# dotchen/LAV

Hardware: NVIDIA H100
Metric: agent_frames_per_s (higher is better)
Workload: dtype fp16 storage, fp32 accumulate (wgmma f16 / mma.sync f16; saturating stores)

## Files before the change

include/lav_b200.h:

```cpp
#ifndef LAV_B200_H
#define LAV_B200_H

#include <stddef.h>
#include <stdint.h>

#ifdef __cplusplus
extern "C" {
#endif

#define LAVB_ABI_VERSION 3

int lavb_abi_version(void);
const char* lavb_last_error(void);
int lavb_device_cc(void);

enum { LAVB_F32 = 0, LAVB_BF16 = 1, LAVB_F16 = 2 };
int lavb_h16_dtype(void);

int lavb_paint(const float* d_pts, int n, int pt_stride,
               const float* d_sem, int ncam, int c_in, int h, int w,
               long long s_cam, long long s_c, long long s_y, long long s_x,
               const float* h_cams, int mode,
               float* d_out, int out_stride, int out_col0, int copy_cols, void* stream);

// ... 160 lines not shown
int lavb_pillar_scatter_max(const float* d_h, const int* d_cell, int m, int c, long long n_cells,
                            float* d_canvas, int* d_argmax, void* stream);
int lavb_pillar_scatter_max_bwd(const float* d_gcanvas, const int* d_argmax, const int* d_cell, int m, int c,
                                float* d_gh, void* stream);

typedef struct {
  const void* in; int in_dtype; int n, hin, win, cin, in_cstride, in_coff;
  void* out; int out_dtype; int hout, wout, cout, out_cstride, out_coff;
  int hog, wog;
  int in_sy, in_sx, out_sy, out_sx, out_oy, out_ox;
  int ntaps; int dy[16]; int dx[16];
  const float* w; const float* bias; const float* scale; const float* shift;
  const void* res; int res_dtype; int res_cstride, res_coff;
  int pre_relu, post_relu, sigmoid;
  int d2s_nout;
} lavb_conv_desc;
int lavb_conv_taps(const lavb_conv_desc* h_desc, void* stream);

int lavb_deconv3x3s2_small(const void* d_in, int dtype, int n, int h, int w, int in_cstride, int groups, int cin_g,
                           const float* d_w, const float* d_bias, const int* h_n_out, const int* h_sigmoid,
                           float* const* h_out_ptrs, void* stream);

int lavb_pool2_affine_relu(const void* d_in, int dtype, int n, int hin, int win, int c, int in_cstride, int in_coff,
                           const float* d_scale, const float* d_shift,
                           void* d_out, int out_cstride, int out_coff, void* stream);

int lavb_rgb_normalize(const void* d_rgb, int src_is_u8_nhwc, int n, int h, int w, void* d_out, int out_dtype,
                       void* stream);

int lavb_stem7x7s2_u8(const void* d_img, int batch, int ncam, int h, int cam_w, const void* d_w, const float* d_bias,
                      const float* h_mean, const float* h_std, void* d_out, void* stream);
int lavb_maxpool3x3s2_nhwc(const void* d_in, int n, int h, int w, int c, void* d_out, void* stream);

size_t lavb_det_peaks_workspace_bytes(int batch, int ncls);
int lavb_det_peaks(const float* d_center, const float* d_box, const float* d_ori, int batch, int h, int w, int ncls,
                   float min_score, int max_det, float* d_packed, void* d_workspace, void* stream);

int lavb_crop_bilinear(const void* d_feat, int dtype, int b, int h, int w, int c, const int* d_frame_idx,
                       const float* d_theta, int k, int crop, void* d_out, void* stream);
int lavb_crop_bilinear_u8(const uint8_t* d_map, int b, int c, int h, int w, const int* d_frame_idx, const float* d_theta,
                          int k, int crop, float* d_out, void* stream);
int lavb_crop_bilinear_bwd(const float* d_gout, int b, int h, int w, int c, const int* d_frame_idx, const float* d_theta,
                           int k, int crop, float* d_gfeat, void* stream);

int lavb_convert(const void* d_src, int src_dtype, void* d_dst, int dst_dtype, long long count, void* stream);

int lavb_conv_umma(const lavb_conv_desc* h_desc, void* stream);

int lavb_conv7x7s2_umma(const void* d_in, int n, int h, int w, int cin, const void* d_w, const float* d_bias, void* d_out,
                        void* stream);

int lavb_conv3x3_umma(const void* d_in, int n, int h, int w, int cin, int stride, const void* d_w, int cout, const float* d_bias,
                      const float* d_scale, const float* d_shift, int pre_relu, void* d_out, void* stream);

typedef struct lavb_conv_pair_desc {
  const void* in; void* out; const void* res;
  int n, h, w, c, dil, post_relu;
  const void* w1; const float* bias1;
  const void* w2; const float* shift2;
} lavb_conv_pair_desc;
int lavb_conv_pair_umma(const lavb_conv_pair_desc* h_desc, void* stream);
int lavb_conv_pair_set_trace(void* d_buf, int tiles_per_cta);

int lavb_erf_stem(const void* d_rgb_u8, int n, int h, int w, const float* h_w27x16, const float* h_scale16,
                  const float* h_shift16, void* d_out, int out_dtype, void* stream);

int lavb_erf_down16(const void* d_in, void* d_out, int n, int h, int w, const float* d_w9, const float* d_st, void* stream);

int lavb_erf_nb16(const void* d_in, void* d_out, int n, int h, int w, const float* d_w4, const float* d_st, void* stream);

int lavb_cast_gru(const float* d_embd, int n, const float* d_wih_t, const float* d_whh_t, const float* d_bih, const float* d_bhh,
                  const float* d_wmlp, const float* d_bmlp, int ncmd, int steps, float* d_out, void* stream);

#ifdef __cplusplus
}
#endif
#endif
```

lav_b200/capi.py:

```python
import ctypes as C
import os

_HERE = os.path.dirname(os.path.abspath(__file__))
LIB_PATH = os.path.join(_HERE, "_lib", "liblavb200.so")

F32, BF16, F16 = 0, 1, 2


class LavbError(RuntimeError):
    pass


class ConvDesc(C.Structure):
    _fields_ = [
        ("inp", C.c_void_p), ("in_dtype", C.c_int), ("n", C.c_int), ("hin", C.c_int), ("win", C.c_int), ("cin", C.c_int),
        ("in_cstride", C.c_int), ("in_coff", C.c_int),
        ("out", C.c_void_p), ("out_dtype", C.c_int), ("hout", C.c_int), ("wout", C.c_int), ("cout", C.c_int),
        ("out_cstride", C.c_int), ("out_coff", C.c_int),
        ("hog", C.c_int), ("wog", C.c_int),
        ("in_sy", C.c_int), ("in_sx", C.c_int), ("out_sy", C.c_int), ("out_sx", C.c_int), ("out_oy", C.c_int), ("out_ox", C.c_int),
        ("ntaps", C.c_int), ("dy", C.c_int * 16), ("dx", C.c_int * 16),
        ("w", C.c_void_p), ("bias", C.c_void_p), ("scale", C.c_void_p), ("shift", C.c_void_p),
        ("res", C.c_void_p), ("res_dtype", C.c_int), ("res_cstride", C.c_int), ("res_coff", C.c_int),
        ("pre_relu", C.c_int), ("post_relu", C.c_int), ("sigmoid", C.c_int), ("d2s_nout", C.c_int),
# ... 84 lines not shown
    "lavb_agent_nav_state_bytes": (C.c_size_t, []),
    "lavb_agent_nav_front": (C.c_int, [C.c_int, C.c_void_p, C.c_void_p, C.c_int, C.c_void_p, C.c_void_p, C.c_void_p, C.c_void_p,
                                       C.c_void_p, C.c_void_p, C.c_void_p, C.c_void_p, C.c_void_p]),
    "lavb_agent_nav_update": (C.c_int, [C.c_int, C.c_void_p, C.c_void_p, C.c_void_p, C.c_void_p, C.c_void_p, C.c_void_p]),
    "lavb_stack_job_poses": (C.c_int, [C.c_void_p, C.c_int, C.c_int, C.c_int, C.c_int, C.c_longlong, C.c_void_p, C.c_void_p,
                                       C.c_void_p]),
    "lavb_agent_view_scratch_bytes": (C.c_size_t, [C.c_int]),
    "lavb_agent_view": (C.c_int, [C.c_void_p, C.c_void_p, C.c_void_p, C.c_int, C.c_longlong, C.c_int, C.c_void_p, C.c_int, C.c_int,
                                  C.c_void_p, C.c_void_p, C.c_void_p, C.c_void_p, C.c_int, C.c_void_p, C.c_void_p, C.c_int, C.c_int,
                                  C.c_void_p, C.c_void_p, C.c_int, C.c_void_p, C.c_void_p, C.POINTER(ViewConfig), C.c_void_p,
                                  C.c_size_t, C.c_void_p, C.c_void_p]),
    "lavb_roof_filter": (C.c_int, [C.c_void_p, C.c_int, C.c_int, C.c_int, C.c_longlong, C.c_void_p, C.c_longlong, C.c_void_p, C.c_int,
                                   C.c_void_p]),
    "lavb_stack_sweep": (C.c_int, [C.c_void_p, C.c_int, C.c_int, C.c_void_p, C.c_float, C.c_float, C.c_int, C.c_int, C.c_int,
                                   C.c_void_p, C.c_void_p]),
    "lavb_pillar_workspace_bytes": (C.c_size_t, [C.c_int, C.c_int, C.c_int]),
    "lavb_pillar_forward": (C.c_int, [C.c_void_p, C.c_int, C.c_int, C.c_void_p, C.c_void_p, C.c_int,
                                      C.c_float, C.c_float, C.c_float, C.c_float, C.c_float, C.c_int, C.c_int,
                                      C.c_void_p, C.c_void_p, C.c_void_p, C.c_int, C.c_void_p, C.c_void_p, C.c_void_p, C.c_int,
                                      C.c_void_p, C.c_int, C.c_void_p, C.c_void_p]),
    "lavb_pillar_sorted_workspace_bytes": (C.c_size_t, [C.c_int, C.c_int, C.c_int, C.c_longlong]),
    "lavb_pillar_forward_sorted": (C.c_int, [C.c_void_p, C.c_int, C.c_int, C.c_void_p, C.c_void_p, C.c_int,
                                             C.c_float, C.c_float, C.c_float, C.c_float, C.c_float, C.c_int, C.c_int,
                                             C.c_void_p, C.c_void_p, C.c_void_p, C.c_int, C.c_void_p, C.c_void_p, C.c_void_p, C.c_int,
                                             C.c_void_p, C.c_int, C.c_void_p, C.c_void_p]),
    "lavb_pillar_decorate": (C.c_int, [C.c_void_p, C.c_int, C.c_int, C.c_void_p, C.c_void_p, C.c_int,
                                       C.c_float, C.c_float, C.c_float, C.c_float, C.c_float, C.c_int, C.c_int,
                                       C.c_void_p, C.c_void_p, C.c_void_p, C.c_void_p, C.c_void_p]),
    "lavb_pillar_scatter_max": (C.c_int, [C.c_void_p, C.c_void_p, C.c_int, C.c_int, C.c_longlong, C.c_void_p, C.c_void_p,
                                          C.c_void_p]),
    "lavb_pillar_scatter_max_bwd": (C.c_int, [C.c_void_p, C.c_void_p, C.c_void_p, C.c_int, C.c_int, C.c_void_p, C.c_void_p]),
    "lavb_conv_taps": (C.c_int, [C.POINTER(ConvDesc), C.c_void_p]),
    "lavb_pool2_affine_relu": (C.c_int, [C.c_void_p, C.c_int, C.c_int, C.c_int, C.c_int, C.c_int, C.c_int, C.c_int,
                                         C.c_void_p, C.c_void_p, C.c_void_p, C.c_int, C.c_int, C.c_void_p]),
    "lavb_rgb_normalize": (C.c_int, [C.c_void_p, C.c_int, C.c_int, C.c_int, C.c_int, C.c_void_p, C.c_int, C.c_void_p]),
    "lavb_convert": (C.c_int, [C.c_void_p, C.c_int, C.c_void_p, C.c_int, C.c_longlong, C.c_void_p]),
    "lavb_stem7x7s2_u8": (C.c_int, [C.c_void_p, C.c_int, C.c_int, C.c_int, C.c_int, C.c_void_p, C.c_void_p, C.c_void_p, C.c_void_p,
                                    C.c_void_p, C.c_void_p]),
    "lavb_erf_stem": (C.c_int, [C.c_void_p, C.c_int, C.c_int, C.c_int, C.c_void_p, C.c_void_p, C.c_void_p, C.c_void_p, C.c_int, C.c_void_p]),
    "lavb_erf_down16": (C.c_int, [C.c_void_p, C.c_void_p, C.c_int, C.c_int, C.c_int, C.c_void_p, C.c_void_p, C.c_void_p]),
    "lavb_erf_nb16": (C.c_int, [C.c_void_p, C.c_void_p, C.c_int, C.c_int, C.c_int, C.c_void_p, C.c_void_p, C.c_void_p]),
    "lavb_conv_pair_umma": (C.c_int, [C.c_void_p, C.c_void_p]),
    "lavb_maxpool3x3s2_nhwc": (C.c_int, [C.c_void_p, C.c_int, C.c_int, C.c_int, C.c_int, C.c_void_p, C.c_void_p]),
    "lavb_det_peaks_workspace_bytes": (C.c_size_t, [C.c_int, C.c_int]),
    "lavb_det_peaks": (C.c_int, [C.c_void_p, C.c_void_p, C.c_void_p, C.c_int, C.c_int, C.c_int, C.c_int, C.c_float, C.c_int,
                                 C.c_void_p, C.c_void_p, C.c_void_p]),
    "lavb_crop_bilinear": (C.c_int, [C.c_void_p, C.c_int, C.c_int, C.c_int, C.c_int, C.c_int, C.c_void_p, C.c_void_p, C.c_int,
                                     C.c_int, C.c_void_p, C.c_void_p]),
    "lavb_crop_bilinear_u8": (C.c_int, [C.c_void_p, C.c_int, C.c_int, C.c_int, C.c_int, C.c_void_p, C.c_void_p, C.c_int, C.c_int,
                                        C.c_void_p, C.c_void_p]),
    "lavb_cast_gru": (C.c_int, [C.c_void_p, C.c_int, C.c_void_p, C.c_void_p, C.c_void_p, C.c_void_p, C.c_void_p, C.c_void_p, C.c_int,
                                C.c_int, C.c_void_p, C.c_void_p]),
    "lavb_conv_pair_set_trace": (C.c_int, [C.c_void_p, C.c_int]),
    "lavb_crop_bilinear_bwd": (C.c_int, [C.c_void_p, C.c_int, C.c_int, C.c_int, C.c_int, C.c_void_p, C.c_void_p, C.c_int, C.c_int,
                                         C.c_void_p, C.c_void_p]),
    "lavb_deconv3x3s2_small": (C.c_int, [C.c_void_p, C.c_int, C.c_int, C.c_int, C.c_int, C.c_int, C.c_int, C.c_int, C.c_void_p,
                                         C.c_void_p, C.c_void_p, C.c_void_p, C.c_void_p, C.c_void_p]),
    "lavb_conv_umma": (C.c_int, [C.POINTER(ConvDesc), C.c_void_p]),
    "lavb_conv7x7s2_umma": (C.c_int, [C.c_void_p, C.c_int, C.c_int, C.c_int, C.c_int, C.c_void_p, C.c_void_p, C.c_void_p,
                                      C.c_void_p]),
    "lavb_conv3x3_umma": (C.c_int, [C.c_void_p, C.c_int, C.c_int, C.c_int, C.c_int, C.c_int, C.c_void_p, C.c_int, C.c_void_p,
                                    C.c_void_p, C.c_void_p, C.c_int, C.c_void_p, C.c_void_p]),
}

_lib = None


def exported_symbols():
    return sorted(_SIGS)


def lib():
    global _lib
    if _lib is None:
        if not os.path.exists(LIB_PATH):
            raise LavbError(f"{LIB_PATH} is missing — run `python -m lav_b200.build` (or __graft_entry__.build()); "
                            "lav_b200 has no CPU fallback")
        handle = C.CDLL(LIB_PATH)
        for name, (res, args) in _SIGS.items():
            fn = getattr(handle, name)
            fn.restype = res
            fn.argtypes = args
        if handle.lavb_abi_version() != 3:
            raise LavbError("liblavb200.so ABI version mismatch")
        _lib = handle
    return _lib


def h16_code():
    return lib().lavb_h16_dtype()


def check(code, what):
    if code != 0:
        raise LavbError(f"{what} failed ({code}): {lib().lavb_last_error().decode()}")
```

lav_b200/csrc/sm90.cuh:

```cuda
#pragma once
#include <cuda.h>
#include <cudaTypedefs.h>
#include "common.cuh"

namespace lavb {
namespace sm90 {

__device__ __forceinline__ uint32_t smem_u32(const void* p) { return (uint32_t)__cvta_generic_to_shared(p); }

__device__ __forceinline__ void proxy_fence_async() { asm volatile("fence.proxy.async.shared::cta;" ::: "memory"); }
__device__ __forceinline__ void bar_sync(int id, int threads) { asm volatile("bar.sync %0, %1;" ::"r"(id), "r"(threads) : "memory"); }

__device__ __forceinline__ void mbar_init(uint32_t bar, uint32_t count) {
  asm volatile("mbarrier.init.shared::cta.b64 [%0], %1;" ::"r"(bar), "r"(count));
}
__device__ __forceinline__ void mbar_expect_tx(uint32_t bar, uint32_t bytes) {
  asm volatile("mbarrier.arrive.expect_tx.shared::cta.b64 _, [%0], %1;" ::"r"(bar), "r"(bytes) : "memory");
}
__device__ __forceinline__ void mbar_arrive(uint32_t bar) {
  asm volatile("mbarrier.arrive.shared::cta.b64 _, [%0];" ::"r"(bar) : "memory");
}
__device__ __forceinline__ void mbar_wait(uint32_t bar, uint32_t parity) {
  uint32_t done;
  do {
    asm volatile(
        "{\n\t.reg .pred p;\n\t"
        "mbarrier.try_wait.parity.shared::cta.b64 p, [%1], %2;\n\t"
        "selp.u32 %0, 1, 0, p;\n\t}"
        : "=r"(done) : "r"(bar), "r"(parity) : "memory");
  } while (!done);
}
__device__ __forceinline__ void tma_load_4d(uint32_t dst, const CUtensorMap* map, uint32_t bar, int c0, int c1, int c2, int c3) {
  asm volatile(
      "cp.async.bulk.tensor.4d.shared::cluster.global.mbarrier::complete_tx::bytes [%0], [%1, {%3, %4, %5, %6}], [%2];"
      ::"r"(dst), "l"(reinterpret_cast<uint64_t>(map)), "r"(bar), "r"(c0), "r"(c1), "r"(c2), "r"(c3) : "memory");
}
__device__ __forceinline__ void tma_load_2d(uint32_t dst, const CUtensorMap* map, uint32_t bar, int c0, int c1) {
  asm volatile(
      "cp.async.bulk.tensor.2d.shared::cluster.global.mbarrier::complete_tx::bytes [%0], [%1, {%3, %4}], [%2];"
      ::"r"(dst), "l"(reinterpret_cast<uint64_t>(map)), "r"(bar), "r"(c0), "r"(c1) : "memory");
}
__device__ __forceinline__ void mbar_arrive(uint32_t bar, uint32_t count) {
  asm volatile("mbarrier.arrive.shared::cta.b64 _, [%0], %1;" ::"r"(bar), "r"(count) : "memory");
}

__device__ __forceinline__ void tma_store_4d(const CUtensorMap* map, uint32_t src, int c0, int c1, int c2, int c3) {
  asm volatile("cp.async.bulk.tensor.4d.global.shared::cta.bulk_group [%0, {%2, %3, %4, %5}], [%1];"
               ::"l"(reinterpret_cast<uint64_t>(map)), "r"(src), "r"(c0), "r"(c1), "r"(c2), "r"(c3) : "memory");
}
__device__ __forceinline__ void bulk_commit() { asm volatile("cp.async.bulk.commit_group;" ::: "memory"); }
template <int N> __device__ __forceinline__ void bulk_wait_read() { asm volatile("cp.async.bulk.wait_group.read %0;" ::"n"(N) : "memory"); }
template <int N> __device__ __forceinline__ void bulk_wait() { asm volatile("cp.async.bulk.wait_group %0;" ::"n"(N) : "memory"); }

inline PFN_cuTensorMapEncodeTiled_v12000 get_encode() {
  static PFN_cuTensorMapEncodeTiled_v12000 fn = nullptr;
  if (!fn) {
    void* p = nullptr;
    cudaDriverEntryPointQueryResult q;
    if (cudaGetDriverEntryPoint("cuTensorMapEncodeTiled", &p, cudaEnableDefault, &q) == cudaSuccess && q == cudaDriverEntryPointSuccess)
      fn = reinterpret_cast<PFN_cuTensorMapEncodeTiled_v12000>(p);
  }
  return fn;
}

__device__ __forceinline__ uint64_t desc_sw128(uint32_t saddr) {
  const uint32_t lo = ((saddr & 0x3FFFFu) >> 4) | (1u << 16);
  const uint32_t hi = (1024u >> 4) | (1u << 30);
  return (uint64_t)lo | ((uint64_t)hi << 32);
}

__device__ __forceinline__ void wgmma_fence() { asm volatile("wgmma.fence.sync.aligned;" ::: "memory"); }
__device__ __forceinline__ void wgmma_commit() { asm volatile("wgmma.commit_group.sync.aligned;" ::: "memory"); }
template <int N> __device__ __forceinline__ void wgmma_wait() { asm volatile("wgmma.wait_group.sync.aligned %0;" ::"n"(N) : "memory"); }
template <int N> __device__ __forceinline__ void acc_fence(float (&d)[N]) {
#pragma unroll
  for (int i = 0; i < N; ++i) asm volatile("" : "+f"(d[i])::"memory");
}

template <int N> __device__ void wgmma(float (&d)[N / 2], uint64_t a, uint64_t b, uint32_t accumulate);

#define LAVB_WG_R0 "%0, %1, %2, %3, %4, %5, %6, %7, %8, %9, %10, %11, %12, %13, %14, %15"
#define LAVB_WG_R1 "%16, %17, %18, %19, %20, %21, %22, %23, %24, %25, %26, %27, %28, %29, %30, %31"
#define LAVB_WG_R2 "%32, %33, %34, %35, %36, %37, %38, %39, %40, %41, %42, %43, %44, %45, %46, %47"
#define LAVB_WG_R3 "%48, %49, %50, %51, %52, %53, %54, %55, %56, %57, %58, %59, %60, %61, %62, %63"
#define LAVB_WG_R4 "%64, %65, %66, %67, %68, %69, %70, %71, %72, %73, %74, %75, %76, %77, %78, %79"
#define LAVB_WG_R5 "%80, %81, %82, %83, %84, %85, %86, %87, %88, %89, %90, %91, %92, %93, %94, %95"
#define LAVB_WG_R6 "%96, %97, %98, %99, %100, %101, %102, %103, %104, %105, %106, %107, %108, %109, %110, %111"
#define LAVB_WG_R7 "%112, %113, %114, %115, %116, %117, %118, %119, %120, %121, %122, %123, %124, %125, %126, %127"
#define LAVB_WG_D4(i) "+f"(d[i]), "+f"(d[i + 1]), "+f"(d[i + 2]), "+f"(d[i + 3])
#define LAVB_WG_D16(i) LAVB_WG_D4(i), LAVB_WG_D4(i + 4), LAVB_WG_D4(i + 8), LAVB_WG_D4(i + 12)
#define LAVB_WGMMA(N, REGS, IA, IB, IP, ...)                                                                         \
  template <> __device__ __forceinline__ void wgmma<N>(float (&d)[N / 2], uint64_t a, uint64_t b, uint32_t accumulate) { \
    asm volatile(                                                                                                      \
        "{\n\t.reg .pred p;\n\t"                                                                                       \
        "setp.ne.b32 p, %" #IP ", 0;\n\t"                                                                              \
        "wgmma.mma_async.sync.aligned.m64n" #N "k16.f32." LAVB_H16_PTX "." LAVB_H16_PTX " "                            \
        "{" REGS "}, %" #IA ", %" #IB ", p, 1, 1, 0, 0;\n\t}"                                                          \
        : __VA_ARGS__                                                                                                  \
        : "l"(a), "l"(b), "r"(accumulate));                                                                            \
  }
LAVB_WGMMA(32, LAVB_WG_R0, 16, 17, 18, LAVB_WG_D16(0))
// ... 29 lines not shown
```

lav_b200/csrc/stem_umma.cu:

```cuda
#include "sm90.cuh"

namespace lavb {
namespace cmajor {

using namespace sm90;

constexpr int kTile = 16;
constexpr int kBlockK = 64;
constexpr int kColBytes = kTile * kBlockK * 2;
constexpr int kThreads = 288;
constexpr int kEpiPitch = 64 * 2 + 16;
constexpr int kEpiPx = 64;
constexpr int kEpiBytes = kEpiPx * kEpiPitch;
constexpr int kMaxCout = 256;
constexpr int kSmemCap = 227 * 1024;

template <int KS, int S, int CO, int SC>
struct Cfg {
  static constexpr int kCols = S == 1 ? kTile + KS - 1 : kTile + (KS - 1) / 2;
  static constexpr int kBoxBytes = kCols * kColBytes;
  static constexpr int kPBytes = SC * S * kBoxBytes;
  static constexpr int kWBytes = CO * kBlockK * 2;
  static constexpr int kN = CO == 64 ? 8 * kTile : 16 * kTile;
  static constexpr int kCtrl = 16 * 32 + 3 * kMaxCout * 4;
  static constexpr int kFixed = 1024  + 2 * kEpiBytes + kCtrl;
  static constexpr int kPStages = kPBytes <= 40 * 1024 ? 3 : 2;
  static constexpr int kWFit = (kSmemCap - kFixed - kPStages * kPBytes) / kWBytes;
  static constexpr int kWStages = kWFit < 12 ? kWFit : 12;
  static constexpr int kSmem = kFixed + kPStages * kPBytes + kWStages * kWBytes;
  static_assert(kWStages >= 3 && kPStages + kWStages <= 32 && kSmem <= kSmemCap, "shared-memory plan");
};

struct Args {
  int ho, wo, cout, kchunks, tiles_x, tiles_per_img, ncol, num_tiles;
  int pre_bias;
  int pre_relu;
  float shift0;
  h16* out;
  const float* bias; const float* scale; const float* shift;
};

template <int KS, int S, int CO, int SC>
__global__ void __launch_bounds__(kThreads, 1) conv_cmajor_kernel(const __grid_constant__ CUtensorMap tmap_x,
                                                                  const __grid_constant__ CUtensorMap tmap_w,
                                                                  const __grid_constant__ Args p) {
  using C = Cfg<KS, S, CO, SC>;
  constexpr int kPStages = C::kPStages, kWStages = C::kWStages, kPBytes = C::kPBytes, kWBytes = C::kWBytes;
  constexpr int kBoxBytes = C::kBoxBytes, kN = C::kN;
  extern __shared__ uint8_t smem_raw[];
  const uint32_t base = (smem_u32(smem_raw) + 1023u) & ~1023u;
  uint8_t* gen = smem_raw + (base - smem_u32(smem_raw));
  const uint32_t wring = base + kPStages * kPBytes;
  const uint32_t epi = wring + kWStages * kWBytes;
  const uint32_t ctrl = epi + 2 * kEpiBytes;
  const uint32_t p_full = ctrl, p_empty = ctrl + 8 * kPStages, w_full = ctrl + 16 * kPStages, w_empty = w_full + 8 * kWStages;
  float* ep_b = reinterpret_cast<float*>(gen + (ctrl - base) + 16 * 32);
  float* ep_s = ep_b + kMaxCout;
  float* ep_t = ep_s + kMaxCout;

  const int warp = threadIdx.x >> 5, lane = threadIdx.x & 31;
  if (threadIdx.x == 0) {
    asm volatile("prefetch.tensormap [%0];" ::"l"(reinterpret_cast<uint64_t>(&tmap_x)) : "memory");
    asm volatile("prefetch.tensormap [%0];" ::"l"(reinterpret_cast<uint64_t>(&tmap_w)) : "memory");
    for (int s = 0; s < kPStages; ++s) { mbar_init(p_full + 8 * s, 1); mbar_init(p_empty + 8 * s, 8); }
    for (int s = 0; s < kWStages; ++s) { mbar_init(w_full + 8 * s, 1); mbar_init(w_empty + 8 * s, 8); }
    asm volatile("fence.mbarrier_init.release.cluster;" ::: "memory");
  }
  for (int c = threadIdx.x; c < p.cout; c += blockDim.x) {
    const float b = p.bias ? __ldg(p.bias + c) : 0.f;
    const float sc = p.scale ? __ldg(p.scale + c) : 1.f;
    const float sh = p.shift ? __ldg(p.shift + c) : p.shift0;
    ep_b[c] = b;
    ep_s[c] = sc;
    ep_t[c] = p.pre_bias ? sh : fmaf(b, sc, sh);
  }
  __syncthreads();
  const int nkg = p.kchunks / SC;

  if (warp == 8) {
    if (lane == 0) {
      int ps = 0, ws = 0; uint32_t pph = 0, wph = 0;
      for (int tile = blockIdx.x; tile < p.num_tiles; tile += gridDim.x) {
        const int col = tile % p.ncol, sp = tile / p.ncol;
        const int img = sp / p.tiles_per_img, r = sp - img * p.tiles_per_img;
        const int y0 = (r / p.tiles_x) * S * kTile - KS / 2, x0 = (r % p.tiles_x) * S * kTile - KS / 2;
        for (int kg = 0; kg < nkg; ++kg) {
          for (int ky = 0; ky < KS; ++ky) {
            mbar_wait(p_empty + 8 * ps, pph ^ 1);
            const uint32_t sp_at = base + ps * kPBytes;
            mbar_expect_tx(p_full + 8 * ps, kPBytes);
            for (int c = 0; c < SC; ++c)
              for (int par = 0; par < S; ++par)
                tma_load_4d(sp_at + (c * S + par) * kBoxBytes, &tmap_x, p_full + 8 * ps, (kg * SC + c) * kBlockK, y0 + ky,
                            x0 + par, img);
            if (++ps == kPStages) { ps = 0; pph ^= 1; }
            for (int kx = 0; kx < KS; ++kx) {
              for (int c = 0; c < SC; ++c) {
                mbar_wait(w_empty + 8 * ws, wph ^ 1);
                mbar_expect_tx(w_full + 8 * ws, kWBytes);
                tma_load_2d(wring + ws * kWBytes, &tmap_w, w_full + 8 * ws, (kg * SC + c) * kBlockK,
                            (KS * ky + kx) * p.cout + col * CO);
                if (++ws == kWStages) { ws = 0; wph ^= 1; }
              }
            }
          }
        }
      }
    }
    return;
  }

  const int wg = warp >> 2;
  const int wtid = threadIdx.x & 127;
  uint8_t* ep = gen + (epi - base) + wg * kEpiBytes;
  const uint32_t a_off = CO == 128 ? wg * (64 * kBlockK * 2) : 0;
  const uint32_t b_off = CO == 64 ? wg * (8 * kColBytes) : 0;
  const int co = 16 * (warp & 3) + (lane >> 2);
  int ps = 0, ws = 0; uint32_t pph = 0, wph = 0;
  float acc[kN / 2];
  for (int tile = blockIdx.x; tile < p.num_tiles; tile += gridDim.x) {
    for (int kg = 0; kg < nkg; ++kg) {
      for (int ky = 0; ky < KS; ++ky) {
        mbar_wait(p_full + 8 * ps, pph);
        const uint32_t sp_at = base + ps * kPBytes + b_off;
        for (int kx = 0; kx < KS; ++kx) {
#pragma unroll
          for (int c = 0; c < SC; ++c) {
            mbar_wait(w_full + 8 * ws, wph);
            const uint64_t a_desc = desc_sw128(wring + ws * kWBytes + a_off);
            const uint64_t b_desc = desc_sw128(sp_at + (c * S + kx % S) * kBoxBytes + (kx / S) * kColBytes);
            const bool first = (kg | ky | kx | c) == 0;
            wgmma_fence();
#pragma unroll
            for (int k = 0; k < kBlockK / 16; ++k)
              wgmma<kN>(acc, a_desc + (uint64_t)(2 * k), b_desc + (uint64_t)(2 * k), (!first || k) ? 1u : 0u);
            wgmma_commit();
            wgmma_wait<1>();
            if (lane == 0 && !first) {
              mbar_arrive(w_empty + 8 * (ws ? ws - 1 : kWStages - 1));
              if (kx == 0 && c == 0) mbar_arrive(p_empty + 8 * (ps ? ps - 1 : kPStages - 1));
            }
            if (++ws == kWStages) { ws = 0; wph ^= 1; }
          }
        }
        if (++ps == kPStages) { ps = 0; pph ^= 1; }
      }
    }
    wgmma_wait<0>();
    acc_fence(acc);
    if (lane == 0) {
      mbar_arrive(w_empty + 8 * (ws ? ws - 1 : kWStages - 1));
      mbar_arrive(p_empty + 8 * (ps ? ps - 1 : kPStages - 1));
    }

    const int col = tile % p.ncol, sp = tile / p.ncol;
    const int img = sp / p.tiles_per_img, r = sp - img * p.tiles_per_img;
    const int oy0 = (r / p.tiles_x) * kTile, ox0 = (r % p.tiles_x) * kTile + (CO == 64 ? 8 * wg : 0);
    const int ch0 = col * CO + (CO == 128 ? 64 * wg : 0);
    const float b0 = ep_b[ch0 + co], b1 = ep_b[ch0 + co + 8];
    const float s0 = ep_s[ch0 + co], s1 = ep_s[ch0 + co + 8];
    const float t0 = ep_t[ch0 + co], t1 = ep_t[ch0 + co + 8];
#pragma unroll
    for (int pass = 0; pass < kN / kEpiPx; ++pass) {
      bar_sync(1 + wg, 128);
#pragma unroll
      for (int i = 8 * pass; i < 8 * pass + 8; ++i)
#pragma unroll
        for (int e = 0; e < 2; ++e) {
          const int px = 8 * i + 2 * (lane & 3) + e - kEpiPx * pass;
          uint8_t* row = ep + px * kEpiPitch;
          float x0 = acc[4 * i + e], x1 = acc[4 * i + 2 + e];
          if (p.pre_bias) { x0 += b0; x1 += b1; }
          if (p.pre_relu) { x0 = fmaxf(x0, 0.f); x1 = fmaxf(x1, 0.f); }
          x0 = fmaf(x0, s0, t0);
          x1 = fmaf(x1, s1, t1);
          *reinterpret_cast<h16*>(row + 2 * co) = float2h16(x0);
          *reinterpret_cast<h16*>(row + 2 * (co + 8)) = float2h16(x1);
        }
      bar_sync(1 + wg, 128);
#pragma unroll
      for (int j = 0; j < kEpiPx * 64 * 2 / 16 / 128; ++j) {
        const int q = wtid + 128 * j, px = q >> 3, piece = q & 7;
        const int n = kEpiPx * pass + px, oy = oy0 + n % kTile, ox = ox0 + n / kTile;
        if (oy < p.ho && ox < p.wo)
          *reinterpret_cast<uint4*>(p.out + (((long long)img * p.ho + oy) * p.wo + ox) * p.cout + ch0 + 8 * piece) =
              *reinterpret_cast<const uint4*>(ep + px * kEpiPitch + 16 * piece);
      }
    }
  }
}

static int encode_maps(const char* who, const void* d_in, int n, int h, int w, int cin, int ks, int s, const void* d_w, int cout,
                       int co, CUtensorMap* tmap_x, CUtensorMap* tmap_w) {
  auto encode = get_encode();
  LAVB_CHECK_ARG(encode != nullptr, "%s: cuTensorMapEncodeTiled not available from the driver", who);
  {
    const int cols = s == 1 ? kTile + ks - 1 : kTile + (ks - 1) / 2;
    cuuint64_t dims[4] = {(cuuint64_t)cin, (cuuint64_t)h, (cuuint64_t)w, (cuuint64_t)n};
    cuuint64_t strides[3] = {(cuuint64_t)w * cin * 2, (cuuint64_t)cin * 2, (cuuint64_t)h * w * cin * 2};
    cuuint32_t box[4] = {(cuuint32_t)kBlockK, (cuuint32_t)(s * kTile), (cuuint32_t)(s * cols), 1};
    cuuint32_t estr[4] = {1, (cuuint32_t)s, (cuuint32_t)s, 1};
    CUresult r = encode(tmap_x, LAVB_TMAP_H16, 4, const_cast<void*>(d_in), dims, strides, box, estr,
                        CU_TENSOR_MAP_INTERLEAVE_NONE, CU_TENSOR_MAP_SWIZZLE_128B, CU_TENSOR_MAP_L2_PROMOTION_L2_256B,
                        CU_TENSOR_MAP_FLOAT_OOB_FILL_NONE);
    LAVB_CHECK_ARG(r == CUDA_SUCCESS, "%s: cuTensorMapEncodeTiled(x) failed with %d", who, (int)r);
  }
  {
    cuuint64_t dims[2] = {(cuuint64_t)cin, (cuuint64_t)ks * ks * cout};
    cuuint64_t strides[1] = {(cuuint64_t)cin * 2};
    cuuint32_t box[2] = {(cuuint32_t)kBlockK, (cuuint32_t)co};
    cuuint32_t estr[2] = {1, 1};
    CUresult r = encode(tmap_w, LAVB_TMAP_H16, 2, const_cast<void*>(d_w), dims, strides, box, estr,
                        CU_TENSOR_MAP_INTERLEAVE_NONE, CU_TENSOR_MAP_SWIZZLE_128B, CU_TENSOR_MAP_L2_PROMOTION_L2_256B,
                        CU_TENSOR_MAP_FLOAT_OOB_FILL_NONE);
    LAVB_CHECK_ARG(r == CUDA_SUCCESS, "%s: cuTensorMapEncodeTiled(w) failed with %d", who, (int)r);
  }
  return 0;
}

template <int KS, int S, int CO, int SC>
static int launch(const CUtensorMap& tmap_x, const CUtensorMap& tmap_w, const Args& a, void* stream) {
  constexpr int smem = Cfg<KS, S, CO, SC>::kSmem;
  LAVB_CUDA_OK(ensure_dyn_smem((const void*)conv_cmajor_kernel<KS, S, CO, SC>, smem));
  conv_cmajor_kernel<KS, S, CO, SC><<<min(a.num_tiles, kNumSMs), kThreads, smem, (cudaStream_t)stream>>>(tmap_x, tmap_w, a);
  LAVB_LAUNCH_OK();
  return 0;
}

static int check_operands(const char* who, const void* d_in, int n, int h, int w, int cin, int taps, const void* d_w, int cout,
                          const float* bias, const float* scale, const float* shift, const void* d_out, int ho, int wo, int co) {
  const auto al = [](const void* q, int a) { return reinterpret_cast<uintptr_t>(q) % a == 0; };
  LAVB_CHECK_ARG(al(d_in, 16) && al(d_w, 16) && al(d_out, 16), "%s: d_in, d_w and d_out must be 16 B aligned", who);
  LAVB_CHECK_ARG(al(bias, 4) && al(scale, 4) && al(shift, 4), "%s: bias, scale and shift must be 4 B aligned", who);
  LAVB_CHECK_ARG((long long)n * ceil_div(ho, kTile) * ceil_div(wo, kTile) * (cout / co) < (1LL << 31), "%s: more than 2^31 tiles", who);
  const long long out_bytes = (long long)n * ho * wo * cout * 2;
  const auto overlap = [&](const void* q, long long bytes) {
    const char *o = static_cast<const char*>(d_out), *c = static_cast<const char*>(q);
    return q && o < c + bytes && c < o + out_bytes;
  };
  LAVB_CHECK_ARG(!overlap(d_in, (long long)n * h * w * cin * 2) && !overlap(d_w, (long long)taps * cout * cin * 2) &&
                 !overlap(bias, 4LL * cout) && !overlap(scale, 4LL * cout) && !overlap(shift, 4LL * cout),
                 "%s: d_out must not overlap d_in, d_w, bias, scale or shift", who);
  return 0;
}

static void tiles(Args& a, int n, int ho, int wo, int cout, int co) {
  a.ho = ho; a.wo = wo; a.cout = cout; a.ncol = cout / co;
  a.tiles_x = ceil_div(wo, kTile);
  a.tiles_per_img = a.tiles_x * ceil_div(ho, kTile);
  a.num_tiles = n * a.tiles_per_img * a.ncol;
}

}
}

using namespace lavb;
using namespace lavb::cmajor;

extern "C" int lavb_conv7x7s2_umma(const void* d_in, int n, int h, int w, int cin, const void* d_w, const float* d_bias,
                                   void* d_out, void* stream) {
  LAVB_CHECK_ARG(d_in && d_w && d_bias && d_out, "conv7x7s2_umma: null operand");
  LAVB_CHECK_ARG(n >= 0 && h >= 7 && w >= 7, "conv7x7s2_umma: bad shape n=%d h=%d w=%d (h, w >= 7)", n, h, w);
  LAVB_CHECK_ARG(cin > 0 && cin % 64 == 0, "conv7x7s2_umma: cin must be a multiple of 64 (got %d)", cin);
  if (n == 0) return 0;
  if (int e = check_operands("conv7x7s2_umma", d_in, n, h, w, cin, 49, d_w, 64, d_bias, nullptr, nullptr, d_out, (h - 1) / 2 + 1,
                             (w - 1) / 2 + 1, 64)) return e;
  CUtensorMap tmap_x, tmap_w;
  if (int e = encode_maps("conv7x7s2_umma", d_in, n, h, w, cin, 7, 2, d_w, 64, 64, &tmap_x, &tmap_w)) return e;
  Args a;
  memset(&a, 0, sizeof(a));
  tiles(a, n, (h - 1) / 2 + 1, (w - 1) / 2 + 1, 64, 64);
  a.kchunks = cin / kBlockK;
  a.pre_bias = 1; a.pre_relu = 1; a.shift0 = -0.f;
  a.out = reinterpret_cast<h16*>(d_out); a.bias = d_bias;
  return launch<7, 2, 64, 1>(tmap_x, tmap_w, a, stream);
}

extern "C" int lavb_conv3x3_umma(const void* d_in, int n, int h, int w, int cin, int stride, const void* d_w, int cout,
                                 const float* d_bias, const float* d_scale, const float* d_shift, int pre_relu, void* d_out,
                                 void* stream) {
  LAVB_CHECK_ARG(d_in && d_w && d_out, "conv3x3_umma: null operand");
  LAVB_CHECK_ARG(n >= 0 && h >= 1 && w >= 1, "conv3x3_umma: bad shape n=%d h=%d w=%d", n, h, w);
  LAVB_CHECK_ARG(stride == 1 || stride == 2, "conv3x3_umma: stride must be 1 or 2 (got %d)", stride);
  LAVB_CHECK_ARG(cin == 64 || cin == 128 || cin == 384, "conv3x3_umma: cin must be 64, 128 or 384 (got %d)", cin);
  LAVB_CHECK_ARG(cout == 64 || cout == 128 || cout == 256, "conv3x3_umma: cout must be 64, 128 or 256 (got %d)", cout);
  LAVB_CHECK_ARG((d_scale == nullptr) == (d_shift == nullptr), "conv3x3_umma: scale and shift come together");
  if (n == 0) return 0;
  const int co = cout == 64 ? 64 : 128;
  if (int e = check_operands("conv3x3_umma", d_in, n, h, w, cin, 9, d_w, cout, d_bias, d_scale, d_shift, d_out, (h - 1) / stride + 1,
                             (w - 1) / stride + 1, co)) return e;
  CUtensorMap tmap_x, tmap_w;
  if (int e = encode_maps("conv3x3_umma", d_in, n, h, w, cin, 3, stride, d_w, cout, co, &tmap_x, &tmap_w)) return e;
  Args a;
  memset(&a, 0, sizeof(a));
  tiles(a, n, (h - 1) / stride + 1, (w - 1) / stride + 1, cout, co);
  a.kchunks = cin / kBlockK;
  a.pre_bias = pre_relu && d_bias != nullptr;
  a.pre_relu = pre_relu != 0;
  a.shift0 = 0.f;
  a.out = reinterpret_cast<h16*>(d_out); a.bias = d_bias; a.scale = d_scale; a.shift = d_shift;
  const int variant = (stride == 2) * 4 + (co == 128) * 2 + (stride == 1 && cin == 128);
  switch (variant) {
    case 0: return launch<3, 1, 64, 1>(tmap_x, tmap_w, a, stream);
    case 1: return launch<3, 1, 64, 2>(tmap_x, tmap_w, a, stream);
    case 2: return launch<3, 1, 128, 1>(tmap_x, tmap_w, a, stream);
    case 3: return launch<3, 1, 128, 2>(tmap_x, tmap_w, a, stream);
    case 4: return launch<3, 2, 64, 1>(tmap_x, tmap_w, a, stream);
    default: return launch<3, 2, 128, 1>(tmap_x, tmap_w, a, stream);
  }
}
```

Before: 1983.

## Use TMA stores with stmatrix staging and resident weights in cmajor conv

For the 3x3 convolution variants, the epilogue now packs results with stmatrix.trans into a 128B-swizzled staging buffer and issues asynchronous TMA tensor stores, double-buffered where shared memory allows. This replaces the per-thread uint4 global stores and the padded staging area. For single-chunk 3x3 stride-1 64-channel convs, all nine weight taps are loaded once and kept resident, which skips the weight ring and its barriers. Optional clock64 trace stamps and a set_trace API are also added. The TMA store relies on the output tensor map's out-of-bounds clipping for partial tiles, and the smaller weight ring may reduce pipelining depth.

```diff
diff --git a/include/lav_b200.h b/include/lav_b200.h
--- a/include/lav_b200.h
+++ b/include/lav_b200.h
@@ -236,6 +236,7 @@
 
 int lavb_conv3x3_umma(const void* d_in, int n, int h, int w, int cin, int stride, const void* d_w, int cout, const float* d_bias,
                       const float* d_scale, const float* d_shift, int pre_relu, void* d_out, void* stream);
+int lavb_conv_cmajor_set_trace(void* d_buf, int tiles_per_cta);
 
 typedef struct lavb_conv_pair_desc {
   const void* in; void* out; const void* res;
diff --git a/lav_b200/capi.py b/lav_b200/capi.py
--- a/lav_b200/capi.py
+++ b/lav_b200/capi.py
@@ -160,6 +160,7 @@
     "lavb_cast_gru": (C.c_int, [C.c_void_p, C.c_int, C.c_void_p, C.c_void_p, C.c_void_p, C.c_void_p, C.c_void_p, C.c_void_p, C.c_int,
                                 C.c_int, C.c_void_p, C.c_void_p]),
     "lavb_conv_pair_set_trace": (C.c_int, [C.c_void_p, C.c_int]),
+    "lavb_conv_cmajor_set_trace": (C.c_int, [C.c_void_p, C.c_int]),
     "lavb_crop_bilinear_bwd": (C.c_int, [C.c_void_p, C.c_int, C.c_int, C.c_int, C.c_int, C.c_void_p, C.c_void_p, C.c_int, C.c_int,
                                          C.c_void_p, C.c_void_p]),
     "lavb_deconv3x3s2_small": (C.c_int, [C.c_void_p, C.c_int, C.c_int, C.c_int, C.c_int, C.c_int, C.c_int, C.c_int, C.c_void_p,
diff --git a/lav_b200/csrc/sm90.cuh b/lav_b200/csrc/sm90.cuh
--- a/lav_b200/csrc/sm90.cuh
+++ b/lav_b200/csrc/sm90.cuh
@@ -47,6 +47,10 @@
 __device__ __forceinline__ void tma_store_4d(const CUtensorMap* map, uint32_t src, int c0, int c1, int c2, int c3) {
   asm volatile("cp.async.bulk.tensor.4d.global.shared::cta.bulk_group [%0, {%2, %3, %4, %5}], [%1];"
                ::"l"(reinterpret_cast<uint64_t>(map)), "r"(src), "r"(c0), "r"(c1), "r"(c2), "r"(c3) : "memory");
+}
+__device__ __forceinline__ void stmatrix_x4_trans(uint32_t addr, uint32_t r0, uint32_t r1, uint32_t r2, uint32_t r3) {
+  asm volatile("stmatrix.sync.aligned.m8n8.x4.trans.shared.b16 [%0], {%1, %2, %3, %4};"
+               ::"r"(addr), "r"(r0), "r"(r1), "r"(r2), "r"(r3) : "memory");
 }
 __device__ __forceinline__ void bulk_commit() { asm volatile("cp.async.bulk.commit_group;" ::: "memory"); }
 template <int N> __device__ __forceinline__ void bulk_wait_read() { asm volatile("cp.async.bulk.wait_group.read %0;" ::"n"(N) : "memory"); }
diff --git a/lav_b200/csrc/stem_umma.cu b/lav_b200/csrc/stem_umma.cu
--- a/lav_b200/csrc/stem_umma.cu
+++ b/lav_b200/csrc/stem_umma.cu
@@ -9,9 +9,9 @@
 constexpr int kBlockK = 64;
 constexpr int kColBytes = kTile * kBlockK * 2;
 constexpr int kThreads = 288;
+constexpr int kEpiPx = 64;
+constexpr int kStageBytes = kEpiPx * 128;
 constexpr int kEpiPitch = 64 * 2 + 16;
-constexpr int kEpiPx = 64;
-constexpr int kEpiBytes = kEpiPx * kEpiPitch;
 constexpr int kMaxCout = 256;
 constexpr int kSmemCap = 227 * 1024;
 
@@ -23,12 +23,18 @@
   static constexpr int kWBytes = CO * kBlockK * 2;
   static constexpr int kN = CO == 64 ? 8 * kTile : 16 * kTile;
   static constexpr int kCtrl = 16 * 32 + 3 * kMaxCout * 4;
-  static constexpr int kFixed = 1024  + 2 * kEpiBytes + kCtrl;
   static constexpr int kPStages = kPBytes <= 40 * 1024 ? 3 : 2;
-  static constexpr int kWFit = (kSmemCap - kFixed - kPStages * kPBytes) / kWBytes;
-  static constexpr int kWStages = kWFit < 12 ? kWFit : 12;
-  static constexpr int kSmem = kFixed + kPStages * kPBytes + kWStages * kWBytes;
-  static_assert(kWStages >= 3 && kPStages + kWStages <= 32 && kSmem <= kSmemCap, "shared-memory plan");
+  static constexpr bool kStoreTma = KS == 3;
+  static constexpr int staging(int bufs) { return kStoreTma ? 2 * bufs * kStageBytes : 2 * kEpiPx * kEpiPitch; }
+  static constexpr int wfit(int bufs) {
+    const int f = (kSmemCap - 1024  - kCtrl - staging(bufs) - kPStages * kPBytes) / kWBytes;
+    return f < 12 ? f : 12;
+  }
+  static constexpr bool kResident = KS == 3 && S == 1 && CO == 64 && SC == 1;
+  static constexpr int kEpiBufs = kStoreTma && (kResident || wfit(2) == wfit(1)) ? 2 : 1;
+  static constexpr int kWStages = wfit(kEpiBufs);
+  static constexpr int kSmem = 1024 + kCtrl + staging(kEpiBufs) + kPStages * kPBytes + kWStages * kWBytes;
+  static_assert(kWStages >= (kResident ? KS * KS : 3) && kPStages + kWStages <= 32 && kSmem <= kSmemCap, "shared-memory plan");
 };
 
 struct Args {
@@ -38,11 +44,17 @@
   float shift0;
   h16* out;
   const float* bias; const float* scale; const float* shift;
+  long long* trace; int trace_tiles;
 };
+#define CMAJOR_STAMP(slot, i, v)                                                                                     \
+  do {                                                                                                              \
+    if (tr && (i) < p.trace_tiles) p.trace[((long long)blockIdx.x * p.trace_tiles + (i)) * 8 + (slot)] = (v);       \
+  } while (0)
 
 template <int KS, int S, int CO, int SC>
 __global__ void __launch_bounds__(kThreads, 1) conv_cmajor_kernel(const __grid_constant__ CUtensorMap tmap_x,
                                                                   const __grid_constant__ CUtensorMap tmap_w,
+                                                                  const __grid_constant__ CUtensorMap tmap_o,
                                                                   const __grid_constant__ Args p) {
   using C = Cfg<KS, S, CO, SC>;
   constexpr int kPStages = C::kPStages, kWStages = C::kWStages, kPBytes = C::kPBytes, kWBytes = C::kWBytes;
@@ -51,8 +63,8 @@
   const uint32_t base = (smem_u32(smem_raw) + 1023u) & ~1023u;
   uint8_t* gen = smem_raw + (base - smem_u32(smem_raw));
   const uint32_t wring = base + kPStages * kPBytes;
-  const uint32_t epi = wring + kWStages * kWBytes;
-  const uint32_t ctrl = epi + 2 * kEpiBytes;
+  const uint32_t stage = wring + kWStages * kWBytes;
+  const uint32_t ctrl = stage + C::staging(C::kEpiBufs);
   const uint32_t p_full = ctrl, p_empty = ctrl + 8 * kPStages, w_full = ctrl + 16 * kPStages, w_empty = w_full + 8 * kWStages;
   float* ep_b = reinterpret_cast<float*>(gen + (ctrl - base) + 16 * 32);
   float* ep_s = ep_b + kMaxCout;
@@ -62,6 +74,7 @@
   if (threadIdx.x == 0) {
     asm volatile("prefetch.tensormap [%0];" ::"l"(reinterpret_cast<uint64_t>(&tmap_x)) : "memory");
     asm volatile("prefetch.tensormap [%0];" ::"l"(reinterpret_cast<uint64_t>(&tmap_w)) : "memory");
+    asm volatile("prefetch.tensormap [%0];" ::"l"(reinterpret_cast<uint64_t>(&tmap_o)) : "memory");
     for (int s = 0; s < kPStages; ++s) { mbar_init(p_full + 8 * s, 1); mbar_init(p_empty + 8 * s, 8); }
     for (int s = 0; s < kWStages; ++s) { mbar_init(w_full + 8 * s, 1); mbar_init(w_empty + 8 * s, 8); }
     asm volatile("fence.mbarrier_init.release.cluster;" ::: "memory");
@@ -76,10 +89,15 @@
   }
   __syncthreads();
   const int nkg = p.kchunks / SC;
+  const bool resident = C::kResident && nkg == 1;
 
   if (warp == 8) {
     if (lane == 0) {
       int ps = 0, ws = 0; uint32_t pph = 0, wph = 0;
+      if (resident) {
+        mbar_expect_tx(w_full, KS * KS * kWBytes);
+        for (int t = 0; t < KS * KS; ++t) tma_load_2d(wring + t * kWBytes, &tmap_w, w_full, 0, t * p.cout);
+      }
       for (int tile = blockIdx.x; tile < p.num_tiles; tile += gridDim.x) {
         const int col = tile % p.ncol, sp = tile / p.ncol;
         const int img = sp / p.tiles_per_img, r = sp - img * p.tiles_per_img;
@@ -94,6 +112,7 @@
                 tma_load_4d(sp_at + (c * S + par) * kBoxBytes, &tmap_x, p_full + 8 * ps, (kg * SC + c) * kBlockK, y0 + ky,
                             x0 + par, img);
             if (++ps == kPStages) { ps = 0; pph ^= 1; }
+            if (resident) continue;
             for (int kx = 0; kx < KS; ++kx) {
               for (int c = 0; c < SC; ++c) {
                 mbar_wait(w_empty + 8 * ws, wph ^ 1);
@@ -111,14 +130,16 @@
   }
 
   const int wg = warp >> 2;
-  const int wtid = threadIdx.x & 127;
-  uint8_t* ep = gen + (epi - base) + wg * kEpiBytes;
+  const bool elect = (threadIdx.x & 127) == 0;
   const uint32_t a_off = CO == 128 ? wg * (64 * kBlockK * 2) : 0;
   const uint32_t b_off = CO == 64 ? wg * (8 * kColBytes) : 0;
   const int co = 16 * (warp & 3) + (lane >> 2);
   int ps = 0, ws = 0; uint32_t pph = 0, wph = 0;
+  const bool tr = p.trace != nullptr && threadIdx.x == 0;
+  if (resident) mbar_wait(w_full, 0);
   float acc[kN / 2];
   for (int tile = blockIdx.x; tile < p.num_tiles; tile += gridDim.x) {
+    const int it = (tile - blockIdx.x) / gridDim.x;
     for (int kg = 0; kg < nkg; ++kg) {
       for (int ky = 0; ky < KS; ++ky) {
         mbar_wait(p_full + 8 * ps, pph);
@@ -126,10 +147,11 @@
         for (int kx = 0; kx < KS; ++kx) {
 #pragma unroll
           for (int c = 0; c < SC; ++c) {
-            mbar_wait(w_full + 8 * ws, wph);
-            const uint64_t a_desc = desc_sw128(wring + ws * kWBytes + a_off);
+            if (!resident) mbar_wait(w_full + 8 * ws, wph);
+            const uint64_t a_desc = desc_sw128(wring + (resident ? KS * ky + kx : ws) * kWBytes + a_off);
             const uint64_t b_desc = desc_sw128(sp_at + (c * S + kx % S) * kBoxBytes + (kx / S) * kColBytes);
             const bool first = (kg | ky | kx | c) == 0;
+            if (first) CMAJOR_STAMP(0, it, clock64());
             wgmma_fence();
 #pragma unroll
             for (int k = 0; k < kBlockK / 16; ++k)
@@ -137,10 +159,10 @@
             wgmma_commit();
             wgmma_wait<1>();
             if (lane == 0 && !first) {
-              mbar_arrive(w_empty + 8 * (ws ? ws - 1 : kWStages - 1));
+              if (!resident) mbar_arrive(w_empty + 8 * (ws ? ws - 1 : kWStages - 1));
               if (kx == 0 && c == 0) mbar_arrive(p_empty + 8 * (ps ? ps - 1 : kPStages - 1));
             }
-            if (++ws == kWStages) { ws = 0; wph ^= 1; }
+            if (!resident && ++ws == kWStages) { ws = 0; wph ^= 1; }
           }
         }
         if (++ps == kPStages) { ps = 0; pph ^= 1; }
@@ -148,8 +170,9 @@
     }
     wgmma_wait<0>();
     acc_fence(acc);
+    CMAJOR_STAMP(1, it, clock64());
     if (lane == 0) {
-      mbar_arrive(w_empty + 8 * (ws ? ws - 1 : kWStages - 1));
+      if (!resident) mbar_arrive(w_empty + 8 * (ws ? ws - 1 : kWStages - 1));
       mbar_arrive(p_empty + 8 * (ps ? ps - 1 : kPStages - 1));
     }
 
@@ -160,38 +183,70 @@
     const float b0 = ep_b[ch0 + co], b1 = ep_b[ch0 + co + 8];
     const float s0 = ep_s[ch0 + co], s1 = ep_s[ch0 + co + 8];
     const float t0 = ep_t[ch0 + co], t1 = ep_t[ch0 + co + 8];
-#pragma unroll
-    for (int pass = 0; pass < kN / kEpiPx; ++pass) {
-      bar_sync(1 + wg, 128);
-#pragma unroll
-      for (int i = 8 * pass; i < 8 * pass + 8; ++i)
-#pragma unroll
-        for (int e = 0; e < 2; ++e) {
-          const int px = 8 * i + 2 * (lane & 3) + e - kEpiPx * pass;
-          uint8_t* row = ep + px * kEpiPitch;
-          float x0 = acc[4 * i + e], x1 = acc[4 * i + 2 + e];
-          if (p.pre_bias) { x0 += b0; x1 += b1; }
-          if (p.pre_relu) { x0 = fmaxf(x0, 0.f); x1 = fmaxf(x1, 0.f); }
-          x0 = fmaf(x0, s0, t0);
-          x1 = fmaf(x1, s1, t1);
-          *reinterpret_cast<h16*>(row + 2 * co) = float2h16(x0);
-          *reinterpret_cast<h16*>(row + 2 * (co + 8)) = float2h16(x1);
-        }
-      bar_sync(1 + wg, 128);
-#pragma unroll
-      for (int j = 0; j < kEpiPx * 64 * 2 / 16 / 128; ++j) {
-        const int q = wtid + 128 * j, px = q >> 3, piece = q & 7;
-        const int n = kEpiPx * pass + px, oy = oy0 + n % kTile, ox = ox0 + n / kTile;
-        if (oy < p.ho && ox < p.wo)
-          *reinterpret_cast<uint4*>(p.out + (((long long)img * p.ho + oy) * p.wo + ox) * p.cout + ch0 + 8 * piece) =
-              *reinterpret_cast<const uint4*>(ep + px * kEpiPitch + 16 * piece);
+    const auto epi = [&](float x, int h) {
+      if (p.pre_bias) x += h ? b1 : b0;
+      if (p.pre_relu) x = fmaxf(x, 0.f);
+      return fmaf(x, h ? s1 : s0, h ? t1 : t0);
+    };
+    if constexpr (!C::kStoreTma) {
+      uint8_t* ep = gen + (stage - base) + wg * kEpiPx * kEpiPitch;
+      const int wtid = threadIdx.x & 127;
+#pragma unroll
+      for (int pass = 0; pass < kN / kEpiPx; ++pass) {
+        bar_sync(1 + wg, 128);
+#pragma unroll
+        for (int i = 8 * pass; i < 8 * pass + 8; ++i)
+#pragma unroll
+          for (int e = 0; e < 2; ++e) {
+            uint8_t* row = ep + (8 * i + 2 * (lane & 3) + e - kEpiPx * pass) * kEpiPitch;
+            *reinterpret_cast<h16*>(row + 2 * co) = float2h16(epi(acc[4 * i + e], 0));
+            *reinterpret_cast<h16*>(row + 2 * (co + 8)) = float2h16(epi(acc[4 * i + 2 + e], 1));
+          }
+        bar_sync(1 + wg, 128);
+        if (pass == kN / kEpiPx - 1) CMAJOR_STAMP(2, it, clock64());
+#pragma unroll
+        for (int j = 0; j < kEpiPx * 64 * 2 / 16 / 128; ++j) {
+          const int q = wtid + 128 * j, px = q >> 3, piece = q & 7;
+          const int n = kEpiPx * pass + px, oy = oy0 + n % kTile, ox = ox0 + n / kTile;
+          if (oy < p.ho && ox < p.wo)
+            *reinterpret_cast<uint4*>(p.out + (((long long)img * p.ho + oy) * p.wo + ox) * p.cout + ch0 + 8 * piece) =
+                *reinterpret_cast<const uint4*>(ep + px * kEpiPitch + 16 * piece);
+        }
+      }
+    } else {
+      const int lrow = 8 * (lane >> 4) + (lane & 7);
+      const uint32_t lchunk = (uint32_t)(((2 * (warp & 3) + ((lane >> 3) & 1)) ^ (lane & 7)) << 4);
+  #pragma unroll
+      for (int pass = 0; pass < kN / kEpiPx; ++pass) {
+        const uint32_t buf = stage + (wg * C::kEpiBufs + pass % C::kEpiBufs) * kStageBytes;
+        if (elect) bulk_wait_read<C::kEpiBufs - 1>();
+        bar_sync(1 + wg, 128);
+  #pragma unroll
+        for (int q = 0; q < 4; ++q) {
+          uint32_t v[4];
+  #pragma unroll
+          for (int m = 0; m < 4; ++m) {
+            const int i = 8 * pass + 2 * q + m / 2, h = m % 2;
+            v[m] = pack_h16(epi(acc[4 * i + 2 * h], h), epi(acc[4 * i + 2 * h + 1], h));
+          }
+          stmatrix_x4_trans(buf + (16 * q + lrow) * 128 + lchunk, v[0], v[1], v[2], v[3]);
+        }
+        proxy_fence_async();
+        bar_sync(1 + wg, 128);
+        if (pass == kN / kEpiPx - 1) CMAJOR_STAMP(2, it, clock64());
+        if (elect) {
+          tma_store_4d(&tmap_o, buf, ch0, oy0, ox0 + 4 * pass, img);
+          bulk_commit();
+        }
       }
     }
-  }
+    CMAJOR_STAMP(3, it, clock64());
+  }
+  if (C::kStoreTma && elect) bulk_wait<0>();
 }
 
 static int encode_maps(const char* who, const void* d_in, int n, int h, int w, int cin, int ks, int s, const void* d_w, int cout,
-                       int co, CUtensorMap* tmap_x, CUtensorMap* tmap_w) {
+                       int co, void* d_out, int ho, int wo, CUtensorMap* tmap_x, CUtensorMap* tmap_w, CUtensorMap* tmap_o) {
   auto encode = get_encode();
   LAVB_CHECK_ARG(encode != nullptr, "%s: cuTensorMapEncodeTiled not available from the driver", who);
   {
@@ -215,14 +270,27 @@
                         CU_TENSOR_MAP_FLOAT_OOB_FILL_NONE);
     LAVB_CHECK_ARG(r == CUDA_SUCCESS, "%s: cuTensorMapEncodeTiled(w) failed with %d", who, (int)r);
   }
+  {
+    cuuint64_t dims[4] = {(cuuint64_t)cout, (cuuint64_t)ho, (cuuint64_t)wo, (cuuint64_t)n};
+    cuuint64_t strides[3] = {(cuuint64_t)wo * cout * 2, (cuuint64_t)cout * 2, (cuuint64_t)ho * wo * cout * 2};
+    cuuint32_t box[4] = {64, (cuuint32_t)kTile, (cuuint32_t)(kEpiPx / kTile), 1};
+    cuuint32_t estr[4] = {1, 1, 1, 1};
+    CUresult r = encode(tmap_o, LAVB_TMAP_H16, 4, d_out, dims, strides, box, estr, CU_TENSOR_MAP_INTERLEAVE_NONE,
+                        CU_TENSOR_MAP_SWIZZLE_128B, CU_TENSOR_MAP_L2_PROMOTION_NONE, CU_TENSOR_MAP_FLOAT_OOB_FILL_NONE);
+    LAVB_CHECK_ARG(r == CUDA_SUCCESS, "%s: cuTensorMapEncodeTiled(out) failed with %d", who, (int)r);
+  }
   return 0;
 }
 
+static long long* g_trace = nullptr;
+static int g_trace_tiles = 0;
+
 template <int KS, int S, int CO, int SC>
-static int launch(const CUtensorMap& tmap_x, const CUtensorMap& tmap_w, const Args& a, void* stream) {
+static int launch(const CUtensorMap& tmap_x, const CUtensorMap& tmap_w, const CUtensorMap& tmap_o, Args a, void* stream) {
   constexpr int smem = Cfg<KS, S, CO, SC>::kSmem;
+  a.trace = g_trace; a.trace_tiles = g_trace_tiles;
   LAVB_CUDA_OK(ensure_dyn_smem((const void*)conv_cmajor_kernel<KS, S, CO, SC>, smem));
-  conv_cmajor_kernel<KS, S, CO, SC><<<min(a.num_tiles, kNumSMs), kThreads, smem, (cudaStream_t)stream>>>(tmap_x, tmap_w, a);
+  conv_cmajor_kernel<KS, S, CO, SC><<<min(a.num_tiles, kNumSMs), kThreads, smem, (cudaStream_t)stream>>>(tmap_x, tmap_w, tmap_o, a);
   LAVB_LAUNCH_OK();
   return 0;
 }
@@ -257,6 +325,12 @@
 using namespace lavb;
 using namespace lavb::cmajor;
 
+extern "C" int lavb_conv_cmajor_set_trace(void* d_buf, int tiles_per_cta) {
+  g_trace = reinterpret_cast<long long*>(d_buf);
+  g_trace_tiles = d_buf ? tiles_per_cta : 0;
+  return 0;
+}
+
 extern "C" int lavb_conv7x7s2_umma(const void* d_in, int n, int h, int w, int cin, const void* d_w, const float* d_bias,
                                    void* d_out, void* stream) {
   LAVB_CHECK_ARG(d_in && d_w && d_bias && d_out, "conv7x7s2_umma: null operand");
@@ -265,15 +339,16 @@
   if (n == 0) return 0;
   if (int e = check_operands("conv7x7s2_umma", d_in, n, h, w, cin, 49, d_w, 64, d_bias, nullptr, nullptr, d_out, (h - 1) / 2 + 1,
                              (w - 1) / 2 + 1, 64)) return e;
-  CUtensorMap tmap_x, tmap_w;
-  if (int e = encode_maps("conv7x7s2_umma", d_in, n, h, w, cin, 7, 2, d_w, 64, 64, &tmap_x, &tmap_w)) return e;
+  CUtensorMap tmap_x, tmap_w, tmap_o;
+  if (int e = encode_maps("conv7x7s2_umma", d_in, n, h, w, cin, 7, 2, d_w, 64, 64, d_out, (h - 1) / 2 + 1, (w - 1) / 2 + 1, &tmap_x,
+                          &tmap_w, &tmap_o)) return e;
   Args a;
   memset(&a, 0, sizeof(a));
   tiles(a, n, (h - 1) / 2 + 1, (w - 1) / 2 + 1, 64, 64);
   a.kchunks = cin / kBlockK;
   a.pre_bias = 1; a.pre_relu = 1; a.shift0 = -0.f;
   a.out = reinterpret_cast<h16*>(d_out); a.bias = d_bias;
-  return launch<7, 2, 64, 1>(tmap_x, tmap_w, a, stream);
+  return launch<7, 2, 64, 1>(tmap_x, tmap_w, tmap_o, a, stream);
 }
 
 extern "C" int lavb_conv3x3_umma(const void* d_in, int n, int h, int w, int cin, int stride, const void* d_w, int cout,
@@ -289,23 +364,25 @@
   const int co = cout == 64 ? 64 : 128;
   if (int e = check_operands("conv3x3_umma", d_in, n, h, w, cin, 9, d_w, cout, d_bias, d_scale, d_shift, d_out, (h - 1) / stride + 1,
                              (w - 1) / stride + 1, co)) return e;
-  CUtensorMap tmap_x, tmap_w;
-  if (int e = encode_maps("conv3x3_umma", d_in, n, h, w, cin, 3, stride, d_w, cout, co, &tmap_x, &tmap_w)) return e;
+  const int ho = (h - 1) / stride + 1, wo = (w - 1) / stride + 1;
+  CUtensorMap tmap_x, tmap_w, tmap_o;
+  if (int e = encode_maps("conv3x3_umma", d_in, n, h, w, cin, 3, stride, d_w, cout, co, d_out, ho, wo, &tmap_x, &tmap_w, &tmap_o))
+    return e;
   Args a;
   memset(&a, 0, sizeof(a));
-  tiles(a, n, (h - 1) / stride + 1, (w - 1) / stride + 1, cout, co);
+  tiles(a, n, ho, wo, cout, co);
   a.kchunks = cin / kBlockK;
   a.pre_bias = pre_relu && d_bias != nullptr;
   a.pre_relu = pre_relu != 0;
   a.shift0 = 0.f;
-  a.out = reinterpret_cast<h16*>(d_out); a.bias = d_bias; a.scale = d_scale; a.shift = d_shift;
+  a.bias = d_bias; a.scale = d_scale; a.shift = d_shift;
   const int variant = (stride == 2) * 4 + (co == 128) * 2 + (stride == 1 && cin == 128);
   switch (variant) {
-    case 0: return launch<3, 1, 64, 1>(tmap_x, tmap_w, a, stream);
-    case 1: return launch<3, 1, 64, 2>(tmap_x, tmap_w, a, stream);
-    case 2: return launch<3, 1, 128, 1>(tmap_x, tmap_w, a, stream);
-    case 3: return launch<3, 1, 128, 2>(tmap_x, tmap_w, a, stream);
-    case 4: return launch<3, 2, 64, 1>(tmap_x, tmap_w, a, stream);
-    default: return launch<3, 2, 128, 1>(tmap_x, tmap_w, a, stream);
-  }
-}
+    case 0: return launch<3, 1, 64, 1>(tmap_x, tmap_w, tmap_o, a, stream);
+    case 1: return launch<3, 1, 64, 2>(tmap_x, tmap_w, tmap_o, a, stream);
+    case 2: return launch<3, 1, 128, 1>(tmap_x, tmap_w, tmap_o, a, stream);
+    case 3: return launch<3, 1, 128, 2>(tmap_x, tmap_w, tmap_o, a, stream);
+    case 4: return launch<3, 2, 64, 1>(tmap_x, tmap_w, tmap_o, a, stream);
+    default: return launch<3, 2, 128, 1>(tmap_x, tmap_w, tmap_o, a, stream);
+  }
+}
```

Result: no change. 1978 (median of 6 runs) (-0.3%).
